# ultravideo/video-stitcher

Measured on AMD Instinct MI355X. Metric: stitched frames/sec, 6x1080p->4K equirect (ms/frame = 1000/value*n_gpus), higher is better.
Workload: dtype u8 in / int16+fp32 pyramid arithmetic; 1 GPU; cfg2: 6x1920x1080 views -> 3840x1920 equirect, spherical, 5 bands, CPW off; a step = 20 passes over a batch of 96 frames per GPU (1920 frames), each pass on 3 HIP stream(s) / contexts, inputs resident in HBM; distinct_frame_sets=8, frames_per_pass=96, streams=3, parallelism=frame-parallel x1

## Files before the change

include/ms_stitch.h:

```cpp
#ifndef MS_STITCH_H
#define MS_STITCH_H

#include <stddef.h>
#include <stdint.h>

#ifdef __cplusplus
extern "C" {
#endif

#define MS_API __attribute__((visibility("default")))

typedef enum ms_status {
    MS_OK = 0,
    MS_ERR_INVALID = -1,
    MS_ERR_UNSUPPORTED = -2,
    MS_ERR_HIP = -3,
    MS_ERR_NO_DEVICE = -4,
    MS_ERR_STATE = -5,
    MS_ERR_NOMEM = -6,
    MS_ERR_COMM = -7
} ms_status;
#define MS_ERR_COMM MS_ERR_COMM

enum { MS_8UC1 = 0, MS_8UC3 = 16, MS_16SC1 = 3, MS_16SC3 = 19, MS_32FC1 = 5 };
// ... 215 lines not shown
MS_API int ms_gain_samples_nv12(ms_ctx *ctx, const ms_image *views_nv12, int stride, void *samples_dev, ms_stream stream);
MS_API int ms_gain_stats_from_samples(ms_ctx *ctx, const void *const *samples_dev, int n, int stride, long long *N_host, long long *S_host, ms_stream stream);
MS_API int ms_track_gains_from_samples(ms_ctx *ctx, const void *const *samples_dev, int n, const ms_gain_track_params *prm, ms_stream stream);

MS_API int ms_set_mesh(ms_ctx *ctx, int view, const float *mesh_x, const float *mesh_y, int N, int M,
                       ms_stream stream);
MS_API int ms_set_meshes(ms_ctx *ctx, const float *mesh_x, const float *mesh_y, int N, int M, ms_stream stream);
MS_API int ms_set_mesh_maps(ms_ctx *ctx, int view, const ms_image *x_mesh, const ms_image *y_mesh, ms_stream stream);

MS_API int ms_stitch(ms_ctx *ctx, int n_frames, const ms_image *views, ms_image *out8u, ms_image *out16s,
                     ms_stream stream);
MS_API int ms_feed(ms_ctx *ctx, int view, const ms_image *img, ms_stream stream);
MS_API int ms_blend(ms_ctx *ctx, ms_image *out8u, ms_image *out16s, ms_stream stream);

MS_API size_t ms_partial_bytes(const ms_ctx *ctx);
MS_API int ms_stitch_partial(ms_ctx *ctx, int n_frames, const ms_image *views, void *partial_out, ms_stream stream);
MS_API int ms_stitch_finish(ms_ctx *ctx, int n_frames, const void *const *partials, int n_partials,
                            ms_image *out8u, ms_image *out16s, ms_stream stream);

MS_API int ms_get_result_mask(ms_ctx *ctx, ms_image *mask);

MS_API int ms_save_tables(ms_ctx *ctx, void *buf, size_t cap, size_t *bytes_out);
MS_API int ms_load_tables(const void *buf, size_t bytes, ms_ctx **out, ms_stream stream);
MS_API int ms_get_band_cells(ms_ctx *ctx, int level, unsigned *owned, unsigned *exclusive, unsigned *general);

typedef struct ms_plan_stats {
    unsigned struct_size;
    int warp_tile_w, warp_tile_h, n_warp_tiles;
    int n_stage1_tiles, n_stage1_reachable;
    int down_tile_w, down_tile_h, n_down_tiles[8];
    int blend_tile_w, blend_tile_h, n_blend_tiles[8];
} ms_plan_stats;
MS_API int ms_get_plan_stats(ms_ctx *ctx, ms_plan_stats *out);

enum { MS_WARP_KERNEL_NONE = 0, MS_WARP_KERNEL_SIMPLE = 1, MS_WARP_KERNEL_SHARED_ALIGNED = 2, MS_WARP_KERNEL_SHARED_UNALIGNED = 3, MS_WARP_KERNEL_PER_FRAME_ALIGNED = 4,
       MS_WARP_KERNEL_PER_FRAME_UNALIGNED = 5, MS_WARP_KERNEL_NV12 = 6, MS_WARP_KERNEL_LDS_STAGED = 7 };
MS_API int ms_get_stitch_kernels(ms_ctx *ctx, int *warp_kernel, int *stage1_kernel);

typedef struct ms_view_geom {
    ms_rect roi;
    int top, left, bottom, right;
    int x_tl, y_tl, x_br, y_br;
} ms_view_geom;
typedef struct ms_pano_geom {
    int num_bands;
    ms_rect dst_roi_final, dst_roi;
    int canvas_x, canvas_y;
} ms_pano_geom;
MS_API int ms_get_view_geom(const ms_ctx *ctx, int view, ms_view_geom *g);
MS_API int ms_get_pano_geom(const ms_ctx *ctx, ms_pano_geom *g);
typedef struct ms_mesh_match {
    float x1, y1;
    float x2, y2;
    int dst;
} ms_mesh_match;

typedef struct ms_mesh_params {
    int mesh_cols, mesh_rows;
    float alphas[4];
    int global_dist;
    float focal_length;
    double compose_scale, work_scale;
    int wrap_around;
    int theta_rule;
    int max_iterations;
    double tolerance;
// ... 223 lines not shown
```

video-stitcher_amd/csrc/compositor.hip:

```cpp
#include <algorithm>
#include <climits>
#include <memory>
#include <mutex>
#include <new>
#include <vector>
#include "common.hpp"
#include "launchers.hpp"
#include "descs.hpp"
#include "ctx.hpp"

namespace ms {

__device__ __forceinline__ void sample3(const uint8_t *__restrict__ src, unsigned sstep, int srows, int scols,
                                        float xc, float yc, float out[3])
{
    const int x1 = f2i_rd(xc), y1 = f2i_rd(yc);
    const int x2 = (int)((unsigned)x1 + 1u), y2 = (int)((unsigned)y1 + 1u);
    const float wx2 = (float)x2 - xc, wx1 = xc - (float)x1;
    const float wy2 = (float)y2 - yc, wy1 = yc - (float)y1;
    const float w[4] = {wx2 * wy2, wx1 * wy2, wx2 * wy1, wx1 * wy1};
    const int xs[4] = {x1, x2, x1, x2};
    const int ys[4] = {y1, y1, y2, y2};
    out[0] = out[1] = out[2] = 0.f;
#pragma unroll
// ... 1223 lines not shown
Bits dilate(const Bits &s, int w, int h, int r)
{
    Bits t((size_t)w * h, 0), o((size_t)w * h, 0);
    for (int y = 0; y < h; ++y)
        for (int x = 0; x < w; ++x) {
            uint8_t m = 0;
            for (int k = std::max(0, x - r); k <= std::min(w - 1, x + r) && !m; ++k) m = s[(size_t)y * w + k];
            t[(size_t)y * w + x] = m;
        }
    for (int y = 0; y < h; ++y)
        for (int x = 0; x < w; ++x) {
            uint8_t m = 0;
            for (int k = std::max(0, y - r); k <= std::min(h - 1, y + r) && !m; ++k) m = t[(size_t)k * w + x];
            o[(size_t)y * w + x] = m;
        }
    return o;
}
Bits half(const Bits &s, int w, int h)
{
    const int hw = (w + 1) / 2, hh = (h + 1) / 2;
    Bits o((size_t)hw * hh, 0);
    for (int y = 0; y < h; ++y)
        for (int x = 0; x < w; ++x)
            if (s[(size_t)y * w + x]) o[(size_t)(y / 2) * hw + x / 2] = 1;
    return o;
}
Bits twice(const Bits &s, int w, int h, int W, int H)
{
    Bits o((size_t)W * H, 0);
    for (int y = 0; y < H; ++y)
        for (int x = 0; x < W; ++x) o[(size_t)y * W + x] = s[(size_t)std::min(y / 2, h - 1) * w + std::min(x / 2, w - 1)];
    return o;
}
bool any_in(const Bits &s, int w, int h, int x0, int y0, int tw, int th)
{
    for (int y = std::max(y0, 0); y < std::min(y0 + th, h); ++y)
        for (int x = std::max(x0, 0); x < std::min(x0 + tw, w); ++x)
            if (s[(size_t)y * w + x]) return true;
    return false;
}

}

template <typename T>
static void xcd_order(std::vector<T> &tiles, int chunk = 0)
{
    const size_t n = tiles.size(), per = (n + 7) / 8;
    if (n < 16) return;
    std::vector<T> out;
    out.reserve(n);
    if (chunk > 0) {
        std::vector<std::vector<T>> q(8);
        for (size_t i = 0; i < n; ++i) q[(i / (size_t)chunk) % 8].push_back(tiles[i]);
        for (size_t i = 0; out.size() < n; ++i)
            for (int k = 0; k < 8; ++k) if (i < q[k].size()) out.push_back(q[k][i]);
        tiles.swap(out);
        return;
    }
    std::vector<char> used(n, 0);
    for (size_t b = 0; out.size() < n; ++b) {
        const size_t src = (b % 8) * per + b / 8;
        if (src < n && !used[src]) { used[src] = 1; out.push_back(tiles[src]); }
        if (b > 16 * n) break;
    }
    for (size_t i = 0; i < n; ++i) if (!used[i]) out.push_back(tiles[i]);
    tiles.swap(out);
// ... 35 lines not shown
        int d = c->cfg.update_mask_margin + 2;
        for (int l = 0; l <= nb; ++l) {
            for (int v = 0; v < N; ++v) {
                const LevelDesc &L = c->h_views[v].lv[l];
                W[v][l] = dilate(W[v][l], L.w, L.h, d);
            }
            d = (d + 1) / 2 + 1;
        }
    }
    const bool windowed = c->col_end > c->col_begin;
    int ra[MAX_LEVELS + 1], rb[MAX_LEVELS + 1];
    std::vector<std::vector<Bits>> Wn_store;
    if (windowed) {
        ra[0] = c->col_begin; rb[0] = c->col_end;
        for (int l = 0; l < nb; ++l) { ra[l + 1] = std::max(ra[l] / 2 - 1, 0); rb[l + 1] = std::min((rb[l] + 1) / 2 + 1, c->pano.qw[l + 1]); }
        Wn_store = W;
        for (int v = 0; v < N; ++v)
            for (int l = 0; l <= nb; ++l) {
                const LevelDesc &L = c->h_views[v].lv[l];
                for (int x = 0; x < L.w; ++x)
                    if (x + L.x_tl < ra[l] || x + L.x_tl >= rb[l])
                        for (int y = 0; y < L.h; ++y) Wn_store[v][l][(size_t)y * L.w + x] = 0;
            }
    }
    const std::vector<std::vector<Bits>> &Wn = windowed ? Wn_store : W;
    double need0 = 0, tot0 = 0;
    for (int v = 0; v < N; ++v) {
        const ViewDesc &V = c->h_views[v];
        for (int l = nb; l >= 0; --l) {
            const LevelDesc &L = V.lv[l];
            Bits n = Wn[v][l];
            if (l >= 1) {
                const LevelDesc &F = V.lv[l - 1];
                Bits u = dilate(half(Wn[v][l - 1], F.w, F.h), L.w, L.h, 1);
                for (size_t i = 0; i < n.size(); ++i) n[i] |= u[i];
            }
            if (l < nb) {
                const LevelDesc &C = V.lv[l + 1];
                Bits d = dilate(twice(Nd[v][l + 1], C.w, C.h, L.w, L.h), L.w, L.h, 2);
                for (size_t i = 0; i < n.size(); ++i) n[i] |= d[i];
            }
            Nd[v][l] = std::move(n);
        }
        tot0 += (double)V.pw * V.ph;
    }
    c->warp_tiled = true;
    for (int v = 0; v < N; ++v) c->warp_tiled = c->warp_tiled && (c->h_views[v].pw % 4 == 0);
    c->warp_tiled = c->warp_tiled && c->cfg.src_width >= 3 && c->cfg.src_height >= 2;
    for (int v = 0; v < N; ++v) c->warp_tiled = c->warp_tiled && c->h_views[v].aw >= 3 && c->h_views[v].ah >= 2;
    {
        std::vector<WarpTile> tiles;
        for (int v = 0; v < N; ++v) {
            if (!((c->own_mask >> v) & 1u)) continue;
            const ViewDesc &V = c->h_views[v];
            for (int y0 = 0; y0 < V.ph; y0 += WARP_TH)
                for (int x0 = 0; x0 < V.pw; x0 += WARP_TW)
                    if (any_in(Nd[v][0], V.pw, V.ph, x0, y0, WARP_TW, WARP_TH)) {
                        WarpTile t{};
                        t.view = (short)v; t.x0 = (short)x0; t.y0 = (short)y0;
                        if (!c->custom_maps && x0 >= V.left && x0 + WARP_TW <= V.left + V.aw && y0 >= V.top && y0 + WARP_TH <= V.top + V.ah) {
                            t.flags |= 4;
                            t.ctab = (int)(c->tab_off[v] + (size_t)(x0 - V.left));
                            t.rtab = (int)(c->tab_off[v] + (size_t)round_up(V.aw, 4) + (size_t)(y0 - V.top));
                        }
                        tiles.push_back(t);
                        need0 += (double)std::min(WARP_TW, V.pw - x0) * std::min(WARP_TH, V.ph - y0);
                    }
        }
        c->needed_mask = 0;
        for (const WarpTile &t : tiles) c->needed_mask |= 1u << t.view;
        for (int v = 0; v < MAX_VIEWS; ++v) c->warp_per_view[v] = 0;
        for (const WarpTile &t : tiles) ++c->warp_per_view[t.view];
        if (!windowed || !c->warp_tiled) c->needed_mask = 0xffffffffu;
        if (c->cfg.raster_tile_order == 0) xcd_order(tiles, dev_knob("MS_XCD_CHUNK_WARP", c->cfg.enable_cpw ? 0 : 32));
        c->n_warp_tiles = (int)tiles.size();
        if (int e = c->warp_tiles.alloc(std::max<size_t>(1, tiles.size()) * sizeof(WarpTile))) return e;
        c->warp_lds_tiles = 0;
        if (!tiles.empty()) {
            MS_HIP(hipMemcpy(c->warp_tiles.p, tiles.data(), tiles.size() * sizeof(WarpTile), hipMemcpyHostToDevice));
            if (c->warp_tiled) {
                k_tile_bbox<<<c->n_warp_tiles, dim3(WARP_BX, std::min(WARP_TH, 256 / WARP_BX))>>>((WarpTile *)c->warp_tiles.p, (const ViewDesc *)c->view_tab.p, c->cfg.src_height, c->cfg.src_width, 0);
                MS_LAUNCH_CHECK();
                MS_HIP(hipMemcpy(tiles.data(), c->warp_tiles.p, tiles.size() * sizeof(WarpTile), hipMemcpyDeviceToHost));
                double sw_sum = 0; int sw_n = 0;
                for (const WarpTile &t : tiles) {
                    if (t.flags & 1) ++c->warp_lds_tiles;
                    if (t.sw > 0) { sw_sum += t.sw; ++sw_n; }
                }
                c->warp_minification = sw_n ? sw_sum / sw_n / WARP_TW : 0.0;
                c->warp_aligned = c->warp_minification > 0 && c->warp_minification < 2.3;
                { const int k = dev_knob("MS_WARP_ALIGNED", -1); if (k >= 0) c->warp_aligned = k != 0; }
                if (dev_knob("MS_DEBUG_PLAN", 0)) {
                    int big = 0, last = 0, interior = 0; long long bytes = 0;
                    for (const WarpTile &t : tiles) {
                        if (t.flags & 1) bytes += 16ll * warp_lds_np(t.sw) * t.sh;
                        else if (t.sw > 0 && 16 * warp_lds_np(t.sw) * t.sh > WA_BUF_BYTES) ++big; else ++last;
                        interior += (t.flags & 4) != 0;
                    }
                    int al = 0;
                    for (const WarpTile &t : tiles) al += (t.flags & 8) != 0;
                    fprintf(stderr, "[plan] warp tiles %zu: staged %d (mean %.0f B), box too large %d, last row / empty %d; interior %d; clear of the last source row %d; "
                                    "minification %.2f -> %s tap reads\n", tiles.size(), c->warp_lds_tiles,
                            c->warp_lds_tiles ? (double)bytes / c->warp_lds_tiles : 0.0, big, last, interior, al, c->warp_minification, c->warp_aligned ? "aligned" : "unaligned");
                }
            }
        }
    }
    c->plan_fraction = tot0 > 0 ? need0 / tot0 : 1.0;
    if (c->cfg.enable_cpw) {
        std::vector<WarpTile> tiles;
        for (int v = 0; v < N; ++v) {
            if (!((c->own_mask >> v) & 1u) || !((c->needed_mask >> v) & 1u)) continue;
            const ViewDesc &V = c->h_views[v];
            Bits a((size_t)V.aw * V.ah, 0);
            for (int y = 0; y < V.ph; ++y)
                for (int x = 0; x < V.pw; ++x)
                    if (Nd[v][0][(size_t)y * V.pw + x]) {
                        int ax = x - V.left, ay = y - V.top;
                        ax = ax < 0 ? -ax - 1 : (ax >= V.aw ? 2 * V.aw - ax - 1 : ax);
                        ay = ay < 0 ? -ay - 1 : (ay >= V.ah ? 2 * V.ah - ay - 1 : ay);
                        a[(size_t)std::min(std::max(ay, 0), V.ah - 1) * V.aw + std::min(std::max(ax, 0), V.aw - 1)] = 1;
                    }
            const int D = CPW_DMAX + 2;
            for (int y0 = 0; y0 < V.ah; y0 += WARP_TH)
                for (int x0 = 0; x0 < V.aw; x0 += WARP_TW) {
                    WarpTile t{}; t.view = (short)v; t.x0 = (short)x0; t.y0 = (short)y0;
                    t.flags = any_in(a, V.aw, V.ah, x0 - D, y0 - D, WARP_TW + 2 * D, WARP_TH + 2 * D) ? 2 : 0;
                    tiles.push_back(t);
                }
        }
        if (dev_knob("MS_DEBUG_PLAN", 0)) { int nf = 0; for (auto &t : tiles) nf += (t.flags & 2) != 0; fprintf(stderr, "[plan] stage-1 tiles %zu, reachable within %d px: %d\n", tiles.size(), CPW_DMAX, nf); }
        {
            std::vector<WarpTile> a, b;
            for (const WarpTile &t : tiles) ((t.flags & 2) ? a : b).push_back(t);
            c->n_stage1_reachable = (int)a.size();
            if (c->cfg.raster_tile_order == 0) { xcd_order(a, dev_knob("MS_XCD_CHUNK_S1", 32)); xcd_order(b, dev_knob("MS_XCD_CHUNK_S1", 32)); }
            tiles = a;
            tiles.insert(tiles.end(), b.begin(), b.end());
        }
        c->n_stage1_tiles = (int)tiles.size();
        for (int v = 0; v < MAX_VIEWS; ++v) c->stage1_per_view[v] = 0;
        for (const WarpTile &t : tiles) ++c->stage1_per_view[t.view];
        if (int e = c->stage1_tiles.alloc(std::max<size_t>(1, tiles.size()) * sizeof(WarpTile))) return e;
        MS_HIP(hipMemcpy(c->stage1_tiles.p, tiles.data(), tiles.size() * sizeof(WarpTile), hipMemcpyHostToDevice));
        if (!tiles.empty() && c->warp_tiled) {
            k_tile_bbox<<<c->n_stage1_tiles, dim3(WARP_BX, std::min(WARP_TH, 256 / WARP_BX))>>>((WarpTile *)c->stage1_tiles.p, (const ViewDesc *)c->view_tab.p, c->cfg.src_height, c->cfg.src_width, 1);
            MS_LAUNCH_CHECK();
            MS_HIP(hipDeviceSynchronize());
        }
    }
    for (int l = 0; l < nb; ++l) {
        std::vector<DownTile> tiles;
        if (c->down_vec[l])
            for (int v = 0; v < N; ++v) {
                if (!((c->own_mask >> v) & 1u)) continue;
                const LevelDesc &Lo = c->h_views[v].lv[l + 1];
                for (int y0 = 0; y0 < Lo.h; y0 += DOWN_TH)
                    for (int x0 = 0; x0 < Lo.w; x0 += DOWN_TW)
                        if (any_in(Nd[v][l + 1], Lo.w, Lo.h, x0, y0, DOWN_TW, DOWN_TH)) tiles.push_back(DownTile{(short)v, 0, (short)x0, (short)y0});
            }
        if (c->cfg.raster_tile_order == 0) xcd_order(tiles, dev_knob(l == 0 ? "MS_XCD_CHUNK_DOWN0" : "MS_XCD_CHUNK_DOWN", 0));
        c->n_down_tiles[l] = (int)tiles.size();
        for (int v = 0; v < MAX_VIEWS; ++v) c->down_per_view[l][v] = 0;
        for (const DownTile &t : tiles) ++c->down_per_view[l][t.view];
        if (int e = c->down_tiles[l].alloc(std::max<size_t>(1, tiles.size()) * sizeof(DownTile))) return e;
        if (!tiles.empty()) MS_HIP(hipMemcpy(c->down_tiles[l].p, tiles.data(), tiles.size() * sizeof(DownTile), hipMemcpyHostToDevice));
    }
    for (int l = 0; l < nb; ++l) {
        std::vector<BlendTile> tiles;
        if (c->blend_vec[l])
            for (int y0 = 0; y0 < c->pano.qh[l]; y0 += BLEND_TH)
                for (int x0 = 0; x0 < c->pano.qw[l]; x0 += BLEND_TW) {
                    if (windowed && (x0 + BLEND_TW <= ra[l] || x0 >= rb[l])) continue;
                    unsigned m = 0;
                    for (int v = 0; v < N; ++v) {
                        const LevelDesc &L = c->h_views[v].lv[l];
                        if (any_in(W[v][l], L.w, L.h, x0 - L.x_tl, y0 - L.y_tl, BLEND_TW, BLEND_TH)) m |= 1u << v;
                    }
                    tiles.push_back(BlendTile{(short)x0, (short)y0, m});
                }
        if (c->cfg.raster_tile_order == 0) xcd_order(tiles, dev_knob(l == 0 ? "MS_XCD_CHUNK_BLEND0" : "MS_XCD_CHUNK_BLEND", (l == 0 && c->pano.qw[0] <= 4096) ? 8 : 0));
        c->n_blend_tiles[l] = (int)tiles.size();
        if (int e = c->blend_tiles[l].alloc(std::max<size_t>(1, tiles.size()) * sizeof(BlendTile))) return e;
        if (!tiles.empty()) MS_HIP(hipMemcpy(c->blend_tiles[l].p, tiles.data(), tiles.size() * sizeof(BlendTile), hipMemcpyHostToDevice));
    }
    c->pure_total = 0;
    for (int l = 0; l < nb; ++l) {
        c->pano.pure[l] = nullptr; c->pano.ppitch[l] = 0; c->pure_off[l] = 0;
        if (!c->blend_vec[l] || sharded_ctx(c) || c->cfg.debug_simple_kernels != 0) continue;
        const int pw_ = div_up(c->pano.qw[l], 64), ph_ = div_up(c->pano.qh[l], 16);
        c->pure_off[l] = c->pure_total + 1;
        c->pano.ppitch[l] = pw_;
        c->pure_total += ((size_t)pw_ * ph_ + 3) & ~(size_t)3;
// ... 1785 lines not shown
    const int pw_ = div_up(c->pano.qw[level], 64), ph_ = div_up(c->pano.qh[level], 16);
    *owned = *exclusive = 0; *general = (unsigned)(pw_ * ph_);
    if (!c->pure_off[level]) return MS_OK;
    std::vector<uint8_t> h((size_t)pw_ * ph_);
    const uint8_t *src = (const uint8_t *)(active == 1 ? c->alt.pure_maps.p : c->pure_maps.p) + (c->pure_off[level] - 1);
    MS_HIP(hipMemcpy(h.data(), src, h.size(), hipMemcpyDeviceToHost));
    *general = 0;
    for (uint8_t b : h) { if (b == 255) ++*general; else if (b == 254) ++*exclusive; else ++*owned; }
    return MS_OK;
}

int ms_get_stitch_kernels(ms_ctx *c, int *warp_kernel, int *stage1_kernel)
{
    if (!c || !warp_kernel || !stage1_kernel) return fail(MS_ERR_INVALID, "null argument");
    *warp_kernel = c->last_warp_kernel; *stage1_kernel = c->last_stage1_kernel;
    return MS_OK;
}

int ms_get_plan_stats(ms_ctx *c, ms_plan_stats *out)
{
    if (!c || !out) return fail(MS_ERR_INVALID, "null argument");
    if (!c->blender_ready) return fail(MS_ERR_STATE, "ms_get_plan_stats: call ms_init_blender first");
    MS_CHECK(out->struct_size == sizeof(ms_plan_stats), "ms_get_plan_stats: struct_size %u, this library's ms_plan_stats has %zu bytes", out->struct_size, sizeof(ms_plan_stats));
    ms_plan_stats s{};
    s.struct_size = (unsigned)sizeof(s);
    s.warp_tile_w = WARP_TW; s.warp_tile_h = WARP_TH; s.n_warp_tiles = c->n_warp_tiles;
    s.n_stage1_tiles = c->n_stage1_tiles; s.n_stage1_reachable = c->n_stage1_reachable;
    s.down_tile_w = DOWN_TW; s.down_tile_h = DOWN_TH; s.blend_tile_w = BLEND_TW; s.blend_tile_h = BLEND_TH;
    for (int l = 0; l < 8 && l < MAX_LEVELS; ++l) { s.n_down_tiles[l] = c->n_down_tiles[l]; s.n_blend_tiles[l] = c->n_blend_tiles[l]; }
    *out = s;
    return MS_OK;
}

static int calib_grid()
{
    int dev = 0, cus = 256;
    (void)hipGetDevice(&dev);
    (void)hipDeviceGetAttribute(&cus, hipDeviceAttributeMultiprocessorCount, dev);
    return 16 * cus;
}

int ms_calib_copy(const void *src, void *dst, size_t bytes, ms_stream stream)
{
    if (int e = require_device()) return e;
    MS_CHECK(src && dst && bytes >= 16 && bytes % 16 == 0 && (((uintptr_t)src | (uintptr_t)dst) & 15) == 0, "ms_calib_copy: 16-byte aligned buffers and size required");
    k_calib_copy<<<calib_grid(), 256, 0, as_stream(stream)>>>((const u32x4_t *)src, (u32x4_t *)dst, bytes / 16);
    MS_LAUNCH_CHECK();
    return MS_OK;
}

int ms_calib_read(const void *src, size_t bytes, ms_stream stream)
{
    if (int e = require_device()) return e;
    MS_CHECK(src && bytes >= 16 && bytes % 16 == 0 && ((uintptr_t)src & 15) == 0, "ms_calib_read: 16-byte aligned buffer and size required");
    unsigned *sink = (unsigned *)device_scratch().get(16);
    if (!sink) return fail(MS_ERR_NOMEM, "ms_calib_read: no device scratch");
    k_calib_read<<<calib_grid(), 256, 0, as_stream(stream)>>>((const u32x4_t *)src, sink, bytes / 16);
    MS_LAUNCH_CHECK();
    return MS_OK;
}

int ms_calib_shape(void *buf, size_t bytes, int shape, ms_stream stream)
{
    if (int e = require_device()) return e;
    MS_CHECK(buf && bytes >= 4096 && bytes % 128 == 0 && ((uintptr_t)buf & 127) == 0 && shape >= 0 && shape <= 2, "ms_calib_shape: 128-byte aligned buffer and size, shape 0..2");
    unsigned *sink = (unsigned *)device_scratch().get(16);
// ... 71 lines not shown
```

video-stitcher_amd/csrc/descs.hpp:

```cpp
#pragma once
#include "common.hpp"

namespace ms {

constexpr int MAX_LEVELS = 8;
constexpr int MAX_VIEWS = 16;
constexpr int MAX_SRC = 192;
constexpr int MAX_FRAMES = 64;
static_assert(MAX_SRC >= MAX_VIEWS, "a source table holds at least one frame of every view");
constexpr int PROJ_MAPS = 3;
static_assert(PROJ_MAPS != MS_PROJ_PLANE && PROJ_MAPS != MS_PROJ_CYLINDRICAL && PROJ_MAPS != MS_PROJ_SPHERICAL, "PROJ_MAPS must not name a projection");

struct LevelDesc {
    int w, h, pitch;
    int x_tl, y_tl;
    long long off;
    const float *wgt;
    int wpitch;
};
struct ViewDesc {
    int aw, ah;
    int top, left;
    int pw, ph;
    float gain;
// ... 11 lines not shown
struct PanoDesc {
    int nb, n_views;
    int qw[MAX_LEVELS], qh[MAX_LEVELS], qpitch[MAX_LEVELS];
    long long coff[MAX_LEVELS];
    long long poff[MAX_LEVELS];
    const float *den[MAX_LEVELS];
    int dpitch[MAX_LEVELS];
    float alpha;
    const uint8_t *mask;
    int mask_pitch;
    int fw, fh;
    int canvas_x, canvas_y, out_w, out_h;
    int i_y0, i_rows;
    const uint8_t *pure[MAX_LEVELS];
    int ppitch[MAX_LEVELS];
};
struct ShardArgs {
    int mode;
    unsigned own_mask;
    int n_parts;
    const int16_t *part[4];
    int16_t *pout;
    long long pstride;
};
struct SrcTable { const uint8_t *p[MAX_SRC]; unsigned step[MAX_SRC]; };
struct SrcAll { const uint8_t *p[MAX_FRAMES * MAX_VIEWS]; unsigned step[MAX_FRAMES * MAX_VIEWS]; };
struct MeshTable { const float *x[MAX_VIEWS]; const float *y[MAX_VIEWS]; int pitch[MAX_VIEWS]; };
struct DispTable { const unsigned *p[MAX_VIEWS]; unsigned limit_bits; };
struct OutTable { uint8_t *p8[MAX_FRAMES]; unsigned step8[MAX_FRAMES]; int16_t *p16[MAX_FRAMES]; unsigned step16[MAX_FRAMES];
                  uint8_t *pi[MAX_FRAMES]; };


struct WarpTile { short view, flags; short x0, y0; short sx0, sy0, sw, sh; int ctab, rtab; };
struct DownTile { short view, pad; short x0, y0; };
struct BlendTile { short x0, y0; unsigned view_mask; };

#ifndef MS_WARP_TW
#define MS_WARP_TW 32
#define MS_WARP_TH 16
#endif
constexpr int WARP_TW = MS_WARP_TW, WARP_TH = MS_WARP_TH;
constexpr int WARP_BX = WARP_TW / 4;
#ifndef MS_DOWN_ROWS
#define MS_DOWN_ROWS 4
#endif
constexpr int DOWN_ROWS = MS_DOWN_ROWS;
constexpr int DOWN_TW = 128, DOWN_TH = 8 * DOWN_ROWS;
constexpr int BLEND_TW = 256, BLEND_TH = 16;

}
```

video-stitcher_amd/csrc/tile_kernels.hpp:

```cpp
#pragma once
#include "descs.hpp"
#ifndef MS_PRIO_WARP
#define MS_PRIO_WARP 1
#endif
#ifndef MS_PRIO_CPW
#define MS_PRIO_CPW 0
#endif
#ifndef MS_PRIO_S1
#define MS_PRIO_S1 0
#endif
#ifndef MS_PRIO_NV12
#define MS_PRIO_NV12 0
#endif
#ifndef MS_PRIO_BLEND
#define MS_PRIO_BLEND 0
#endif
#define MS_PRIO_LOADS(K) do { if ((K) == 1 || (K) == 3) __builtin_amdgcn_s_setprio(3); else if ((K) == 2) __builtin_amdgcn_s_setprio(0); } while (0)
#define MS_PRIO_RELOADS(K) do { if ((K) == 1) __builtin_amdgcn_s_setprio(3); else if ((K) == 2) __builtin_amdgcn_s_setprio(0); } while (0)
#define MS_PRIO_MATH(K)  do { if ((K) == 1 || (K) == 3) __builtin_amdgcn_s_setprio(0); else if ((K) == 2) __builtin_amdgcn_s_setprio(3); } while (0)

namespace ms {

__device__ __forceinline__ int reflect_fast(int i, int len)
{
// ... 1255 lines not shown
    Down7 r;
    r.a[0] = d0 & 0x00ff00ffu; r.a[1] = d1 & 0x00ff00ffu; r.a[2] = d2 & 0x00ff00ffu; r.a[3] = d3 & 0x00ff00ffu;
    r.a[4] = (d0 >> 8) & 0x00ff00ffu; r.a[5] = (d1 >> 8) & 0x00ff00ffu; r.a[6] = (d2 >> 8) & 0x00ff00ffu;
    if (8 * t + 8 >= w) r.a[3] = r.a[2] >> 16;
    return r;
}
__device__ __forceinline__ unsigned rne8_pk(unsigned s)
{
    const unsigned t = pk_lshr16(s, 8) & 0x00010001u;
    return pk_lshr16(s + t + 0x007f007fu, 8);
}
__device__ __forceinline__ unsigned down_hpass(const Down7 &v)
{
    const unsigned e01 = __builtin_amdgcn_alignbyte(v.a[1], v.a[0], 2), e12 = v.a[1], e23 = __builtin_amdgcn_alignbyte(v.a[2], v.a[1], 2);
    const unsigned e34 = v.a[2], e45 = __builtin_amdgcn_alignbyte(v.a[3], v.a[2], 2);
    const unsigned o01 = __builtin_amdgcn_alignbyte(v.a[5], v.a[4], 2), o12 = v.a[5], o23 = __builtin_amdgcn_alignbyte(v.a[6], v.a[5], 2), o34 = v.a[6];
    const unsigned s01 = mad6(e12, e01 + e23 + 4u * (o01 + o12));
    const unsigned s23 = mad6(e34, e23 + e45 + 4u * (o23 + o34));
    return __builtin_amdgcn_perm(rne8_pk(s23), rne8_pk(s01), 0x06040200u);
}

template <bool L0>
__global__ void __launch_bounds__(256) __attribute__((amdgpu_waves_per_eu(6, 8))) k_down_t(const DownTile *__restrict__ tiles, const ViewDesc *__restrict__ views, int l,
                                                const uint8_t *__restrict__ gin, long long in_stride,
                                                uint8_t *__restrict__ gout, long long out_stride)
{
    const DownTile T = tiles[blockIdx.x];
    const int c = blockIdx.y, f = blockIdx.z, v = T.view;
    const int ty = (int)threadIdx.y;
    const LevelDesc &Li = views[v].lv[l], &Lo = views[v].lv[l + 1];
    constexpr int RO = DOWN_ROWS, RI = 2 * RO + 3;
    const int t = (T.x0 >> 2) + (int)threadIdx.x;
    const int y = T.y0 + RO * ty;
    if (4 * t >= Lo.w || y >= Lo.h) return;
    const uint8_t *in = gin + (size_t)f * in_stride + Li.off + (size_t)c * Li.h * Li.pitch;
    const int nrow = min(RO, Lo.h - y);
    const int sy = 2 * y, last = Li.h - 1;
    int ridx[RI];
    ridx[0] = abs(sy - 2); ridx[1] = abs(sy - 1); ridx[2] = sy;
#pragma unroll
    for (int j = 3; j < RI; ++j) { const int r = sy + j - 2; ridx[j] = r > last ? 2 * last - r : r; }
#pragma unroll
    for (int j = 5; j < RI; ++j) if (j > 2 * nrow + 2) ridx[j] = ridx[4];
    Row11u8 raw[RI];
#pragma unroll
    for (int j = 0; j < RI; ++j) raw[j] = fetch_row11(in + (size_t)ridx[j] * Li.pitch, t, Li.w);
    Down7 r[RI];
#pragma unroll
    for (int j = 0; j < RI; ++j) r[j] = down_row(raw[j], t, Li.w);
    uint8_t *out = gout + (size_t)f * out_stride + Lo.off + (size_t)c * Lo.h * Lo.pitch + (size_t)y * Lo.pitch + 4 * t;
#pragma unroll
    for (int o = 0; o < RO; ++o) {
        Down7 vv;
#pragma unroll
        for (int k = 0; k < 7; ++k) vv.a[k] = mad6(r[2 * o + 2].a[k], (r[2 * o].a[k] + r[2 * o + 4].a[k]) + 4u * (r[2 * o + 1].a[k] + r[2 * o + 3].a[k]));
        if (o < nrow) *reinterpret_cast<unsigned *>(out + (size_t)o * Lo.pitch) = down_hpass(vv);
    }
}

}
```

video-stitcher_amd/msstitch.py:

```python
import ctypes as C
import os

_HERE = os.path.dirname(os.path.abspath(__file__))
LIB_PATH = os.path.join(_HERE, "libmsstitch.so")

MS_8UC1, MS_8UC3, MS_16SC1, MS_16SC3, MS_32FC1 = 0, 16, 3, 19, 5
BORDER_CONSTANT, BORDER_REFLECT = 0, 2
INTER_NEAREST, INTER_LINEAR = 0, 1
INTER_LINEAR_FIXPT = 0x101
PROJ_PLANE, PROJ_CYLINDRICAL, PROJ_SPHERICAL = 0, 1, 2
MAPS_ANALYTIC, MAPS_CUSTOM, MAPS_LENS = 0, 1, 2
SEAM_VORONOI, SEAM_DP = 0, 1
DP_MAX_SIDE = 4096
LENS_NONE, LENS_BROWN, LENS_FISHEYE = 0, 1, 2
LENS_CYL_MAX_ELEVATION_DEG = 80
MAPS_MIN_WIDTH, MAPS_MIN_HEIGHT, MAPS_MAX_SIDE = 3, 2, 31744


class MsError(RuntimeError):
    pass


class Image(C.Structure):
    _fields_ = [("data", C.c_void_p), ("step", C.c_size_t), ("cols", C.c_int), ("rows", C.c_int), ("type", C.c_int)]
# ... 71 lines not shown

class ViewJob(C.Structure):
    _fields_ = [("map_x", Image), ("map_y", Image), ("dst_x", C.c_int), ("dst_y", C.c_int)]


class SeamParams(C.Structure):
    _fields_ = [("seam_scale", C.c_double), ("seam_warp_scale", C.c_float), ("dilate", C.c_int), ("estimate_gains", C.c_int)]


class ViewGeom(C.Structure):
    _fields_ = [("roi", Rect)] + [(n, C.c_int) for n in ("top", "left", "bottom", "right", "x_tl", "y_tl", "x_br", "y_br")]


class PanoGeom(C.Structure):
    _fields_ = [("num_bands", C.c_int), ("dst_roi_final", Rect), ("dst_roi", Rect), ("canvas_x", C.c_int), ("canvas_y", C.c_int)]


class RigParams(C.Structure):
    _fields_ = [("num_views", C.c_int), ("src_width", C.c_int), ("src_height", C.c_int), ("hfov_deg", C.c_double),
                ("work_megapix", C.c_double), ("seam_megapix", C.c_double), ("compose_megapix", C.c_double)]


class Rig(C.Structure):
    _fields_ = [("work_scale", C.c_double), ("seam_scale", C.c_double), ("seam_work_aspect", C.c_double), ("compose_scale", C.c_double),
                ("compose_work_aspect", C.c_double), ("warped_image_scale", C.c_float), ("seam_warp_scale", C.c_float),
                ("compose_warp_scale", C.c_float), ("resize_input", C.c_int), ("compose_width", C.c_int), ("compose_height", C.c_int),
                ("K_compose", (C.c_float * 9) * 16), ("K_seam", (C.c_float * 9) * 16), ("R", (C.c_float * 9) * 16)]


class PlanStats(C.Structure):
    _fields_ = [("struct_size", C.c_uint), ("warp_tile_w", C.c_int), ("warp_tile_h", C.c_int), ("n_warp_tiles", C.c_int), ("n_stage1_tiles", C.c_int),
                ("n_stage1_reachable", C.c_int), ("down_tile_w", C.c_int), ("down_tile_h", C.c_int), ("n_down_tiles", C.c_int * 8),
                ("blend_tile_w", C.c_int), ("blend_tile_h", C.c_int), ("n_blend_tiles", C.c_int * 8)]


class MeshMatch(C.Structure):
    _fields_ = [("x1", C.c_float), ("y1", C.c_float), ("x2", C.c_float), ("y2", C.c_float), ("dst", C.c_int)]


class MeshParams(C.Structure):
    _fields_ = [("mesh_cols", C.c_int), ("mesh_rows", C.c_int), ("alphas", C.c_float * 4), ("global_dist", C.c_int),
                ("focal_length", C.c_float), ("compose_scale", C.c_double), ("work_scale", C.c_double), ("wrap_around", C.c_int),
                ("theta_rule", C.c_int), ("max_iterations", C.c_int), ("tolerance", C.c_double)]


class MeshInfo(C.Structure):
    _fields_ = [("rows", C.c_int), ("cols", C.c_int), ("nnz", C.c_int), ("iterations", C.c_int), ("error", C.c_double)]


class RigMatch(C.Structure):
    _fields_ = [("view_a", C.c_int), ("view_b", C.c_int), ("a", C.c_double * 3), ("b", C.c_double * 3)]


class RigRefineParams(C.Structure):
    _fields_ = [("struct_size", C.c_uint), ("anchor_view", C.c_int), ("huber_rad", C.c_double), ("max_iters", C.c_int), ("step_tol", C.c_double),
                ("min_pair_matches", C.c_int)]


class RigRefineInfo(C.Structure):
    _fields_ = [("iterations", C.c_int), ("stop_reason", C.c_int), ("cost_initial", C.c_double), ("cost_final", C.c_double), ("matches_used", C.c_int),
                ("pairs_used", C.c_int), ("pairs_ignored", C.c_int), ("outliers", C.c_int), ("max_rotation_rad", C.c_double)]


RIG_CONVERGED, RIG_STALLED, RIG_ITERATION_LIMIT = 0, 1, 2


# ... 86 lines not shown
GAIN_SAMPLES_HEADER_WORDS = 16
GAIN_MAX_SAMPLE_BUFS = 4


EXPORTS = [
    "ms_last_error", "ms_version", "ms_device_count", "ms_remap", "ms_resize_linear", "ms_convert_scale_8u", "ms_convert",
    "ms_copy_make_border", "ms_pyr_down", "ms_pyr_up", "ms_subtract_16s", "ms_add_16s", "ms_add_src_weight_32f",
    "ms_normalize_using_weight_32f", "ms_add_src_weight_16s", "ms_normalize_using_weight_16s", "ms_compare_gt_32f", "ms_compare_eq_8u", "ms_set_zero_masked_16sc3",
    "ms_bitwise_and_8u", "ms_dilate3x3_8u", "ms_build_warp_maps", "ms_custom_resize_32f", "ms_warp_roi", "ms_result_roi",
    "ms_calibrate_cameras", "ms_num_bands_rule", "ms_orb_default_params", "ms_orb_detect_and_compute", "ms_find_homography_ransac", "ms_feature_mask",
    "ms_create", "ms_destroy", "ms_set_camera", "ms_set_gain", "ms_build_maps", "ms_build_masks", "ms_set_mask",
    "ms_init_blender", "ms_set_mesh", "ms_set_meshes", "ms_set_mesh_maps", "ms_stitch", "ms_get_result_mask", "ms_get_band_cells", "ms_get_view_geom",
    "ms_get_pano_geom", "ms_get_maps", "ms_get_mask", "ms_get_weight_level", "ms_get_mesh_maps", "ms_stitch_timed",
    "ms_selftest_divide", "ms_selftest_divide_range", "ms_calib_copy", "ms_calib_read", "ms_mesh_triangle_masks", "ms_bgr_to_i420", "ms_calibrate_seam", "ms_nv12_to_bgr", "ms_partial_bytes", "ms_stitch_partial", "ms_stitch_finish", "ms_selftest_cvt_u8", "ms_init_feather", "ms_get_mesh_displacement", "ms_set_mesh_interp", "ms_feed", "ms_blend", "ms_update_mask",
    "ms_mesh_default_params", "ms_mesh_saliency", "ms_create_mesh", "ms_knn_match_hamming2", "ms_bgr_to_i420_batch", "ms_bgr_to_gray", "ms_stitch_i420", "ms_get_i420_rows", "ms_get_col_window", "ms_get_needed_views", "ms_consume_i420", "ms_resize_linear_batch", "ms_nv12_to_bgr_batch",
    "ms_save_tables", "ms_load_tables", "ms_calib_shape", "ms_stitch_nv12", "ms_get_plan_stats", "ms_get_stitch_kernels",
    "ms_set_active_views", "ms_get_active_views",
    "ms_gain_track_default_params", "ms_gain_stats", "ms_track_gains", "ms_get_gains",
    "ms_stitch_nv12_i420", "ms_gain_stats_nv12", "ms_track_gains_nv12", "ms_nv12_resize_linear_batch",
    "ms_gain_partial_bytes", "ms_get_gain_views", "ms_gain_stats_partial", "ms_gain_stats_partial_nv12", "ms_track_gains_from_partials", "ms_get_gain_track_counters",
    "ms_gain_samples_bytes", "ms_get_view_shard", "ms_get_gain_sample_views", "ms_gain_samples", "ms_gain_samples_nv12", "ms_gain_stats_from_samples", "ms_track_gains_from_samples",
    "ms_voronoi_seams", "ms_estimate_gains",
    "ms_set_maps", "ms_get_map_source",
    "ms_lens_check", "ms_lens_project", "ms_set_lens", "ms_get_lens", "ms_build_warp_maps_lens", "ms_warp_roi_lens",
    "ms_warper_rays", "ms_rig_refine_default_params", "ms_rig_accumulate", "ms_refine_rig_rotations", "ms_refine_rig",
    "ms_dp_seams", "ms_set_seam_finder", "ms_get_seam_finder",
    "ms_focals_from_homography", "ms_estimate_rig", "ms_rig_focal_default_params", "ms_rig_focal_accumulate", "ms_refine_rig_cameras", "ms_refine_rig_focals",
    "ms_pair_match_default_params", "ms_match_pairs", "ms_biggest_component", "ms_wave_correct",
    "ms_find_homography_ransac_batch",
    "ms_orb_detect_and_compute_batch",
    "ms_list_match_default_params", "ms_match_lists", "ms_feature_inputs_batch",
    "ms_lens_unproject", "ms_lens_unproject_points", "ms_rig_lens_accumulate", "ms_refine_rig_cameras_lens", "ms_refine_rig_focals_lens",
    "ms_look_at_view", "ms_cube_face_view", "ms_get_pano_frame", "ms_build_view_maps", "ms_reproject",
]

_lib = None


def load():
    global _lib
    if _lib is None:
        if not os.path.exists(LIB_PATH):
            raise MsError("libmsstitch.so not built (run video-stitcher_amd/build.sh or __graft_entry__.build()); "
                          "there is no CPU fallback")
        _lib = C.CDLL(os.environ.get("MSSTITCH_LIB", LIB_PATH))
        _lib.ms_last_error.restype = C.c_char_p
        _lib.ms_version.restype = C.c_char_p
    return _lib


def _chk(code):
    if code < 0:
        raise MsError("msstitch error %d: %s" % (code, load().ms_last_error().decode()))
    return code


_TYPES = {}


def _torch():
    import torch
    if not _TYPES:
        _TYPES.update({(torch.uint8, 1): MS_8UC1, (torch.uint8, 3): MS_8UC3, (torch.int16, 1): MS_16SC1,
                       (torch.int16, 3): MS_16SC3, (torch.float32, 1): MS_32FC1})
    return torch

# ... 1110 lines not shown
        m = Image()
        _chk(load().ms_get_weight_level(self._ctx, view, level, C.byref(m)))
        return tensor_of(m)

    def mesh_maps(self, view):
        xm, ym = Image(), Image()
        _chk(load().ms_get_mesh_maps(self._ctx, view, C.byref(xm), C.byref(ym)))
        return tensor_of(xm), tensor_of(ym)

    def result_mask(self):
        m = Image()
        _chk(load().ms_get_result_mask(self._ctx, C.byref(m)))
        return tensor_of(m)

    def band_cells(self, level):
        a, b, c = C.c_uint(), C.c_uint(), C.c_uint()
        _chk(load().ms_get_band_cells(self._ctx, level, C.byref(a), C.byref(b), C.byref(c)))
        return a.value, b.value, c.value

    def stitch_kernels(self):
        names = {0: "none", 1: "simple", 2: "shared_aligned", 3: "shared_unaligned", 4: "per_frame_aligned", 5: "per_frame_unaligned", 6: "nv12", 7: "lds_staged"}
        a, b = C.c_int(), C.c_int()
        _chk(load().ms_get_stitch_kernels(self._ctx, C.byref(a), C.byref(b)))
        return names[a.value], names[b.value]

    def plan_stats(self):
        st = PlanStats()
        st.struct_size = C.sizeof(PlanStats)
        _chk(load().ms_get_plan_stats(self._ctx, C.byref(st)))
        return {"warp_tile": (st.warp_tile_w, st.warp_tile_h), "n_warp_tiles": st.n_warp_tiles, "n_stage1_tiles": st.n_stage1_tiles,
                "n_stage1_reachable": st.n_stage1_reachable, "down_tile": (st.down_tile_w, st.down_tile_h), "n_down_tiles": list(st.n_down_tiles),
                "blend_tile": (st.blend_tile_w, st.blend_tile_h), "n_blend_tiles": list(st.n_blend_tiles)}

    def _tables(self, frames, out8u, out16s):
        n_frames = len(frames)
        views = (Image * (n_frames * self.n))()
        k = 0
        for fr in frames:
            assert len(fr) == self.n
            for t in fr:
                views[k] = img(t) if t is not None else Image(); k += 1
        o8 = o16 = None
        if out8u is not None:
            o8 = (Image * n_frames)(*[img(t) if t is not None else Image() for t in out8u])
        if out16s is not None:
            o16 = (Image * n_frames)(*[img(t) if t is not None else Image() for t in out16s])
        return n_frames, views, o8, o16

    def stitch(self, frames, out8u=None, out16s=None):
        n, views, o8, o16 = self._tables(frames, out8u, out16s)
        _chk(load().ms_stitch(self._ctx, n, views, o8, o16, _stream()))

    def stitch_nv12(self, frames_nv12, out8u=None, out16s=None):
        n, views, o8, o16 = self._tables(frames_nv12, out8u, out16s)
        _chk(load().ms_stitch_nv12(self._ctx, n, views, o8, o16, _stream()))

    def prepared_nv12(self, frames_nv12, out8u=None, out16s=None):
        n, views, o8, o16 = self._tables(frames_nv12, out8u, out16s)
        fn, ctx = load().ms_stitch_nv12, self._ctx

        def run(stream=None):
            _chk(fn(ctx, n, views, o8, o16, stream if stream is not None else _stream()))
        run.keepalive = (frames_nv12, out8u, out16s, views, o8, o16)
        return run

    def prepared(self, frames, out8u=None, out16s=None):
# ... 233 lines not shown
```

Baseline: 36980 frames/s.

## Tighten pyramid needed-pixel masks with exact filter taps and trim reduce tiles

Computes the needed-pixel masks per pyramid level from the exact pyrDown/pyrUp tap footprints (reflect-101 and clamp borders) rather than a conservative dilate of half/twice. The looser mask is kept only to choose warp tiles. Reduce (downsample) tiles are now built per row band from runs of needed columns and carry an end column xe, so the kernel stops at xe instead of the level width. This cuts reduce work on unneeded columns, but correctness depends on the exact tap masks matching the kernels. Also adds a plan-tile query API and debug prints.

Result: faster. 37960 frames/s, median of 6 (+2.7%).

```diff
diff --git a/include/ms_stitch.h b/include/ms_stitch.h
--- a/include/ms_stitch.h
+++ b/include/ms_stitch.h
@@ -271,6 +271,8 @@
     int blend_tile_w, blend_tile_h, n_blend_tiles[8];
 } ms_plan_stats;
 MS_API int ms_get_plan_stats(ms_ctx *ctx, ms_plan_stats *out);
+typedef struct ms_plan_tile { int view, x0, y0, xe; } ms_plan_tile;
+MS_API int ms_get_plan_tiles(ms_ctx *ctx, int list, ms_plan_tile *out, int cap, int *count);
 
 enum { MS_WARP_KERNEL_NONE = 0, MS_WARP_KERNEL_SIMPLE = 1, MS_WARP_KERNEL_SHARED_ALIGNED = 2, MS_WARP_KERNEL_SHARED_UNALIGNED = 3, MS_WARP_KERNEL_PER_FRAME_ALIGNED = 4,
        MS_WARP_KERNEL_PER_FRAME_UNALIGNED = 5, MS_WARP_KERNEL_NV12 = 6, MS_WARP_KERNEL_LDS_STAGED = 7 };
diff --git a/video-stitcher_amd/csrc/compositor.hip b/video-stitcher_amd/csrc/compositor.hip
--- a/video-stitcher_amd/csrc/compositor.hip
+++ b/video-stitcher_amd/csrc/compositor.hip
@@ -1279,6 +1279,53 @@
         for (int x = 0; x < W; ++x) o[(size_t)y * W + x] = s[(size_t)std::min(y / 2, h - 1) * w + std::min(x / 2, w - 1)];
     return o;
 }
+int reflect101(int i, int n)
+{
+    const int last = n - 1;
+    return std::abs(last - std::abs(last - i)) % n;
+}
+int pyrup_idx(int i, int n) { i = std::abs(i); return i < n - 1 ? i : n - 1; }
+Bits down_taps(const Bits &s, int cw, int ch, int w, int h)
+{
+    Bits t((size_t)w * ch, 0), o((size_t)w * h, 0);
+    for (int i = 0; i < ch; ++i)
+        for (int j = 0; j < cw; ++j)
+            if (s[(size_t)i * cw + j])
+                for (int k = -2; k <= 2; ++k) t[(size_t)i * w + reflect101(std::abs(2 * j + k), w)] = 1;
+    for (int i = 0; i < ch; ++i)
+        for (int x = 0; x < w; ++x)
+            if (t[(size_t)i * w + x])
+                for (int k = -2; k <= 2; ++k) o[(size_t)reflect101(std::abs(2 * i + k), h) * w + x] = 1;
+    return o;
+}
+Bits up_taps(const Bits &s, int w, int h, int cw, int ch)
+{
+    Bits t((size_t)cw * h, 0), o((size_t)cw * ch, 0);
+    for (int y = 0; y < h; ++y)
+        for (int x = 0; x < w; ++x)
+            if (s[(size_t)y * w + x])
+                for (int k = (x & 1) ? 0 : -1; k <= 1; ++k) t[(size_t)y * cw + pyrup_idx(x / 2 + k, cw)] = 1;
+    for (int y = 0; y < h; ++y)
+        for (int j = 0; j < cw; ++j)
+            if (t[(size_t)y * cw + j])
+                for (int k = (y & 1) ? 0 : -1; k <= 1; ++k) o[(size_t)pyrup_idx(y / 2 + k, ch) * cw + j] = 1;
+    return o;
+}
+template <class Emit>
+void row_tiles(const Bits &s, int w, int h, int y0, int tw, int th, Emit emit)
+{
+    std::vector<uint8_t> col((size_t)w, 0);
+    for (int y = y0; y < std::min(y0 + th, h); ++y)
+        for (int x = 0; x < w; ++x) col[x] |= s[(size_t)y * w + x];
+    for (int x = 0; x < w;) {
+        if (!col[x]) { ++x; continue; }
+        int end = x + 1;
+        for (int k = x + 1; k < w && k < end + tw; ++k) if (col[k]) end = k + 1;
+        const int xe = (end + 3) & ~3;
+        for (int x0 = x & ~3; x0 < end; x0 += tw) emit(x0, std::min(x0 + tw, xe));
+        x = end;
+    }
+}
 bool any_in(const Bits &s, int w, int h, int x0, int y0, int tw, int th)
 {
     for (int y = std::max(y0, 0); y < std::min(y0 + th, h); ++y)
@@ -1380,17 +1427,39 @@
             Bits n = Wn[v][l];
             if (l >= 1) {
                 const LevelDesc &F = V.lv[l - 1];
+                Bits u = up_taps(Wn[v][l - 1], F.w, F.h, L.w, L.h);
+                for (size_t i = 0; i < n.size(); ++i) n[i] |= u[i];
+            }
+            if (l < nb) {
+                const LevelDesc &C = V.lv[l + 1];
+                Bits d = down_taps(Nd[v][l + 1], C.w, C.h, L.w, L.h);
+                for (size_t i = 0; i < n.size(); ++i) n[i] |= d[i];
+            }
+            Nd[v][l] = std::move(n);
+        }
+        tot0 += (double)V.pw * V.ph;
+    }
+    std::vector<Bits> Nw(N);
+    for (int v = 0; v < N; ++v) {
+        const ViewDesc &V = c->h_views[v];
+        Bits m;
+        for (int l = nb; l >= 0; --l) {
+            const LevelDesc &L = V.lv[l];
+            Bits n = Wn[v][l];
+            if (l >= 1) {
+                const LevelDesc &F = V.lv[l - 1];
                 Bits u = dilate(half(Wn[v][l - 1], F.w, F.h), L.w, L.h, 1);
                 for (size_t i = 0; i < n.size(); ++i) n[i] |= u[i];
             }
             if (l < nb) {
                 const LevelDesc &C = V.lv[l + 1];
-                Bits d = dilate(twice(Nd[v][l + 1], C.w, C.h, L.w, L.h), L.w, L.h, 2);
+                Bits d = dilate(twice(m, C.w, C.h, L.w, L.h), L.w, L.h, 2);
                 for (size_t i = 0; i < n.size(); ++i) n[i] |= d[i];
             }
-            Nd[v][l] = std::move(n);
-        }
-        tot0 += (double)V.pw * V.ph;
+            m = std::move(n);
+        }
+        Nw[v] = std::move(m);
+        if ((c->own_mask >> v) & 1u) for (uint8_t b : Nw[v]) need0 += b;
     }
     c->warp_tiled = true;
     for (int v = 0; v < N; ++v) c->warp_tiled = c->warp_tiled && (c->h_views[v].pw % 4 == 0);
@@ -1398,12 +1467,13 @@
     for (int v = 0; v < N; ++v) c->warp_tiled = c->warp_tiled && c->h_views[v].aw >= 3 && c->h_views[v].ah >= 2;
     {
         std::vector<WarpTile> tiles;
+        long long warp_lanes = 0;
         for (int v = 0; v < N; ++v) {
             if (!((c->own_mask >> v) & 1u)) continue;
             const ViewDesc &V = c->h_views[v];
             for (int y0 = 0; y0 < V.ph; y0 += WARP_TH)
                 for (int x0 = 0; x0 < V.pw; x0 += WARP_TW)
-                    if (any_in(Nd[v][0], V.pw, V.ph, x0, y0, WARP_TW, WARP_TH)) {
+                    if (any_in(Nw[v], V.pw, V.ph, x0, y0, WARP_TW, WARP_TH)) {
                         WarpTile t{};
                         t.view = (short)v; t.x0 = (short)x0; t.y0 = (short)y0;
                         if (!c->custom_maps && x0 >= V.left && x0 + WARP_TW <= V.left + V.aw && y0 >= V.top && y0 + WARP_TH <= V.top + V.ah) {
@@ -1412,7 +1482,7 @@
                             t.rtab = (int)(c->tab_off[v] + (size_t)round_up(V.aw, 4) + (size_t)(y0 - V.top));
                         }
                         tiles.push_back(t);
-                        need0 += (double)std::min(WARP_TW, V.pw - x0) * std::min(WARP_TH, V.ph - y0);
+                        warp_lanes += std::min(WARP_TW, V.pw - x0) / 4 * std::min(WARP_TH, V.ph - y0);
                     }
         }
         c->needed_mask = 0;
@@ -1447,6 +1517,7 @@
                     }
                     int al = 0;
                     for (const WarpTile &t : tiles) al += (t.flags & 8) != 0;
+                    fprintf(stderr, "[plan] needed level-0 px %.0f of %.0f padded; lanes that write %lld (4 px each)\n", need0, tot0, warp_lanes);
                     fprintf(stderr, "[plan] warp tiles %zu: staged %d (mean %.0f B), box too large %d, last row / empty %d; interior %d; clear of the last source row %d; "
                                     "minification %.2f -> %s tap reads\n", tiles.size(), c->warp_lds_tiles,
                             c->warp_lds_tiles ? (double)bytes / c->warp_lds_tiles : 0.0, big, last, interior, al, c->warp_minification, c->warp_aligned ? "aligned" : "unaligned");
@@ -1463,7 +1534,7 @@
             Bits a((size_t)V.aw * V.ah, 0);
             for (int y = 0; y < V.ph; ++y)
                 for (int x = 0; x < V.pw; ++x)
-                    if (Nd[v][0][(size_t)y * V.pw + x]) {
+                    if (Nw[v][(size_t)y * V.pw + x]) {
                         int ax = x - V.left, ay = y - V.top;
                         ax = ax < 0 ? -ax - 1 : (ax >= V.aw ? 2 * V.aw - ax - 1 : ax);
                         ay = ay < 0 ? -ay - 1 : (ay >= V.ah ? 2 * V.ah - ay - 1 : ay);
@@ -1499,14 +1570,22 @@
     }
     for (int l = 0; l < nb; ++l) {
         std::vector<DownTile> tiles;
+        long long down_lanes = 0;
         if (c->down_vec[l])
             for (int v = 0; v < N; ++v) {
                 if (!((c->own_mask >> v) & 1u)) continue;
                 const LevelDesc &Lo = c->h_views[v].lv[l + 1];
                 for (int y0 = 0; y0 < Lo.h; y0 += DOWN_TH)
-                    for (int x0 = 0; x0 < Lo.w; x0 += DOWN_TW)
-                        if (any_in(Nd[v][l + 1], Lo.w, Lo.h, x0, y0, DOWN_TW, DOWN_TH)) tiles.push_back(DownTile{(short)v, 0, (short)x0, (short)y0});
+                    row_tiles(Nd[v][l + 1], Lo.w, Lo.h, y0, DOWN_TW, DOWN_TH, [&](int x0, int xe) {
+                        tiles.push_back(DownTile{(short)v, (short)xe, (short)x0, (short)y0});
+                        down_lanes += (xe - x0) / 4 * div_up(std::min(DOWN_TH, Lo.h - y0), DOWN_ROWS);
+                    });
             }
+        if (dev_knob("MS_DEBUG_PLAN", 0)) {
+            long long need = 0;
+            for (int v = 0; v < N; ++v) if ((c->own_mask >> v) & 1u) for (uint8_t b : Nd[v][l + 1]) need += b;
+            fprintf(stderr, "[plan] reduce %d -> %d: tiles %zu, lanes that write %lld (4 x %d px each), needed px of level %d %lld\n", l, l + 1, tiles.size(), down_lanes, DOWN_ROWS, l + 1, need);
+        }
         if (c->cfg.raster_tile_order == 0) xcd_order(tiles, dev_knob(l == 0 ? "MS_XCD_CHUNK_DOWN0" : "MS_XCD_CHUNK_DOWN", 0));
         c->n_down_tiles[l] = (int)tiles.size();
         for (int v = 0; v < MAX_VIEWS; ++v) c->down_per_view[l][v] = 0;
@@ -3358,6 +3437,25 @@
     return MS_OK;
 }
 
+int ms_get_plan_tiles(ms_ctx *c, int list, ms_plan_tile *out, int cap, int *count)
+{
+    if (!c || !count || cap < 0 || (cap > 0 && !out)) return fail(MS_ERR_INVALID, "ms_get_plan_tiles: null argument or negative capacity");
+    if (!c->blender_ready) return fail(MS_ERR_STATE, "ms_get_plan_tiles: call ms_init_blender first");
+    MS_CHECK(list >= 0 && list <= c->pano.nb, "ms_get_plan_tiles: list %d not in [0, %d]", list, c->pano.nb);
+    if (list == 0) {
+        std::vector<WarpTile> h((size_t)c->n_warp_tiles);
+        if (!h.empty()) MS_HIP(hipMemcpy(h.data(), c->warp_tiles.p, h.size() * sizeof(WarpTile), hipMemcpyDeviceToHost));
+        for (int i = 0; i < (int)h.size() && i < cap; ++i) out[i] = ms_plan_tile{h[i].view, h[i].x0, h[i].y0, std::min(h[i].x0 + WARP_TW, c->h_views[h[i].view].pw)};
+        *count = (int)h.size();
+    } else {
+        std::vector<DownTile> h((size_t)c->n_down_tiles[list - 1]);
+        if (!h.empty()) MS_HIP(hipMemcpy(h.data(), c->down_tiles[list - 1].p, h.size() * sizeof(DownTile), hipMemcpyDeviceToHost));
+        for (int i = 0; i < (int)h.size() && i < cap; ++i) out[i] = ms_plan_tile{h[i].view, h[i].x0, h[i].y0, h[i].xe};
+        *count = (int)h.size();
+    }
+    return MS_OK;
+}
+
 static int calib_grid()
 {
     int dev = 0, cus = 256;
diff --git a/video-stitcher_amd/csrc/descs.hpp b/video-stitcher_amd/csrc/descs.hpp
--- a/video-stitcher_amd/csrc/descs.hpp
+++ b/video-stitcher_amd/csrc/descs.hpp
@@ -67,7 +67,7 @@
 
 
 struct WarpTile { short view, flags; short x0, y0; short sx0, sy0, sw, sh; int ctab, rtab; };
-struct DownTile { short view, pad; short x0, y0; };
+struct DownTile { short view, xe; short x0, y0; };
 struct BlendTile { short x0, y0; unsigned view_mask; };
 
 #ifndef MS_WARP_TW
diff --git a/video-stitcher_amd/csrc/tile_kernels.hpp b/video-stitcher_amd/csrc/tile_kernels.hpp
--- a/video-stitcher_amd/csrc/tile_kernels.hpp
+++ b/video-stitcher_amd/csrc/tile_kernels.hpp
@@ -1311,7 +1311,7 @@
     constexpr int RO = DOWN_ROWS, RI = 2 * RO + 3;
     const int t = (T.x0 >> 2) + (int)threadIdx.x;
     const int y = T.y0 + RO * ty;
-    if (4 * t >= Lo.w || y >= Lo.h) return;
+    if (4 * t >= T.xe || y >= Lo.h) return;
     const uint8_t *in = gin + (size_t)f * in_stride + Li.off + (size_t)c * Li.h * Li.pitch;
     const int nrow = min(RO, Lo.h - y);
     const int sy = 2 * y, last = Li.h - 1;
diff --git a/video-stitcher_amd/msstitch.py b/video-stitcher_amd/msstitch.py
--- a/video-stitcher_amd/msstitch.py
+++ b/video-stitcher_amd/msstitch.py
@@ -127,6 +127,10 @@
     _fields_ = [("struct_size", C.c_uint), ("warp_tile_w", C.c_int), ("warp_tile_h", C.c_int), ("n_warp_tiles", C.c_int), ("n_stage1_tiles", C.c_int),
                 ("n_stage1_reachable", C.c_int), ("down_tile_w", C.c_int), ("down_tile_h", C.c_int), ("n_down_tiles", C.c_int * 8),
                 ("blend_tile_w", C.c_int), ("blend_tile_h", C.c_int), ("n_blend_tiles", C.c_int * 8)]
+
+
+class PlanTile(C.Structure):
+    _fields_ = [("view", C.c_int), ("x0", C.c_int), ("y0", C.c_int), ("xe", C.c_int)]
 
 
 class MeshMatch(C.Structure):
@@ -279,6 +283,7 @@
     "ms_list_match_default_params", "ms_match_lists", "ms_feature_inputs_batch",
     "ms_lens_unproject", "ms_lens_unproject_points", "ms_rig_lens_accumulate", "ms_refine_rig_cameras_lens", "ms_refine_rig_focals_lens",
     "ms_look_at_view", "ms_cube_face_view", "ms_get_pano_frame", "ms_build_view_maps", "ms_reproject",
+    "ms_get_plan_tiles",
 ]
 
 _lib = None
@@ -1455,6 +1460,14 @@
                 "n_stage1_reachable": st.n_stage1_reachable, "down_tile": (st.down_tile_w, st.down_tile_h), "n_down_tiles": list(st.n_down_tiles),
                 "blend_tile": (st.blend_tile_w, st.blend_tile_h), "n_blend_tiles": list(st.n_blend_tiles)}
 
+    def plan_tiles(self, which):
+        import numpy as np
+        n = C.c_int()
+        _chk(load().ms_get_plan_tiles(self._ctx, int(which), None, 0, C.byref(n)))
+        buf = (PlanTile * max(n.value, 1))()
+        _chk(load().ms_get_plan_tiles(self._ctx, int(which), buf, n.value, C.byref(n)))
+        return np.array([(t.view, t.x0, t.y0, t.xe) for t in buf[:n.value]], dtype=np.int64).reshape(-1, 4)
+
     def _tables(self, frames, out8u, out16s):
         n_frames = len(frames)
         views = (Image * (n_frames * self.n))()
```
